# starkware-libs/stark-perpetual

Measured on AMD Instinct MI355X. Metric: pedersen_hashes_per_sec, higher is better.
Workload: dtype u32x9; 1 GPU; 2^16-leaf Pedersen Merkle rebuild per GPU (BASELINE.json configs[1]), 63 rebuilds in lockstep; tree_height=16, leaves_per_gpu=65536, calls_per_region=28, streams=2, window_bits=26, combine=none

## Files before the change

### stark-perpetual_amd/csrc/pedersen.hip

```cpp
#include <cstdlib>
#include <cstring>
#include <map>
#include <vector>

#include "context.hpp"
#include "quad.hpp"

#ifndef SP_ACC_WAVES
#define SP_ACC_WAVES 1
#endif

namespace sp {

struct raw_aff {
  u256 x, y;
};
__device__ __forceinline__ raw_aff ld_raw(const aff_packed* e) {
  const uint4* q = reinterpret_cast<const uint4*>(e);
  const uint4 a = q[0], b = q[1], c = q[2], d = q[3];
  raw_aff r;
  r.x.w[0] = a.x; r.x.w[1] = a.y; r.x.w[2] = a.z; r.x.w[3] = a.w;
  r.x.w[4] = b.x; r.x.w[5] = b.y; r.x.w[6] = b.z; r.x.w[7] = b.w;
  r.y.w[0] = c.x; r.y.w[1] = c.y; r.y.w[2] = c.z; r.y.w[3] = c.w;
  r.y.w[4] = d.x; r.y.w[5] = d.y; r.y.w[6] = d.z; r.y.w[7] = d.w;
  return r;
}
__device__ __forceinline__ aff unpack_raw(const raw_aff& t) {
  aff r;
  r.x = fe_unpack(t.x);
  r.y = fe_unpack(t.y);
  return r;
}

struct bits512 {
  uint32_t w[16];
};
__device__ __forceinline__ bits512 concat_xy(const u256& x, const u256& y) {
  bits512 s;
// ... 35 lines not shown
__device__ __forceinline__ int window_width(int g, int w0, int log2e) { return g == 0 ? w0 : log2e + 1; }
__device__ __forceinline__ int window_start(int g, int w0, int log2e) {
  return g == 0 ? 0 : w0 + (g - 1) * (log2e + 1);
}
__device__ __forceinline__ aff signed_aff(const raw_aff& t, bool negative) {
  aff q = unpack_raw(t);
  if (negative) q.y = fe_neg(q.y);
  return q;
}

__device__ __forceinline__ void store_limbs(int32_t* base, size_t n, size_t e, const fe& v) {
#pragma unroll
  for (int k = 0; k < NL; ++k) base[(size_t)k * n + e] = v.l[k];
}
__device__ __forceinline__ fe load_limbs(const int32_t* base, size_t n, size_t e) {
  fe v;
#pragma unroll
  for (int k = 0; k < NL; ++k) v.l[k] = base[(size_t)k * n + e];
  return v;
}

__device__ __forceinline__ void operand_pointers(const uint64_t* x, const uint64_t* y, size_t xstride,
                                                 size_t ystride, const int2* __restrict__ src, size_t e,
                                                 const uint64_t*& fx, const uint64_t*& fy) {
  if (src == nullptr) {
    fx = x + 4 * e * xstride;
    fy = y + 4 * e * ystride;
  } else {
    const int2 s = src[e];
    fx = s.x >= 0 ? x + 4 * (size_t)s.x : y;
    fy = s.y >= 0 ? x + 4 * (size_t)s.y : y;
  }
}

__device__ __forceinline__ void
bulk_accumulate(const uint64_t* __restrict__ x, const uint64_t* __restrict__ y, size_t xstride,
                size_t ystride, size_t n, const aff_packed* __restrict__ ped, int w0, int log2e,
                int nwin, int32_t* __restrict__ sX, int32_t* __restrict__ sZZ,
                uint8_t* __restrict__ status, unsigned* __restrict__ flag,
                const int2* __restrict__ src, size_t plane, size_t e) {
  if (e >= n) return;
  const uint64_t *fx, *fy;
  operand_pointers(x, y, xstride, ystride, src, e, fx, fy);
  u256 sx = ld_u256(fx);
  u256 sy = ld_u256(fy);
  uint8_t st = SP_HASH_OK;
  if (!u256_lt(sx, U256_P) || !u256_lt(sy, U256_P)) {
    st = SP_HASH_OUT_OF_RANGE;
#pragma unroll
    for (int i = 0; i < 8; ++i) { sx.w[i] = 0; sy.w[i] = 0; }
  }
  bits512 str = concat_xy(sx, sy);
  auto next_window = [&](int g) {
    return window_entry(ped, g, pop_bits(str, window_width(g, w0, log2e)), w0, log2e);
  };
  const raw_aff e0 = ld_raw(next_window(0).entry);
  window_ref r1 = next_window(1 < nwin ? 1 : 0);
  raw_aff n1 = ld_raw(r1.entry);
  bool neg1 = r1.negative, neg2 = false;
  raw_aff n2 = n1;
  if (nwin > 2) {
    const window_ref r2 = next_window(2);
    n2 = ld_raw(r2.entry);
    neg2 = r2.negative;
  }
  xyzz acc;
  int first = 1;
  if (nwin > 2) {
    const aff q1 = signed_aff(n1, neg1);
    n1 = n2;
    neg1 = neg2;
    if (3 < nwin) {
      const window_ref r = next_window(3);
      n2 = ld_raw(r.entry);
      neg2 = r.negative;
    }
    acc = xyzz_mmadd(unpack_raw(e0), q1);
    first = 2;
  } else {
    acc = xyzz_from_aff(unpack_raw(e0));
  }
  for (int i = first; i + 1 < nwin; ++i) {
    const aff q = signed_aff(n1, neg1);
    n1 = n2;
    neg1 = neg2;
    if (i + 2 < nwin) {
      const window_ref r = next_window(i + 2);
      n2 = ld_raw(r.entry);
      neg2 = r.negative;
    }
    acc = xyzz_madd(acc, q);
  }
  if (nwin > 1) {
    fe X3, ZZ3;
    xyzz_madd_x_only(acc, signed_aff(n1, neg1), X3, ZZ3);
    store_limbs(sX, plane, e, X3);
    store_limbs(sZZ, plane, e, ZZ3);
  } else {
    store_limbs(sX, plane, e, acc.X);
    store_limbs(sZZ, plane, e, acc.ZZ);
  }
  if (st != SP_HASH_OK) {
    if (status) status[e] = st;
    if (flag) atomicOr(flag, (unsigned)st);
  } else if (status) {
    status[e] = SP_HASH_OK;
  }
}

__global__ void __launch_bounds__(256, SP_ACC_WAVES)
ped_accumulate_kernel(const uint64_t* __restrict__ x, const uint64_t* __restrict__ y, size_t xstride,
                      size_t ystride, size_t n, const aff_packed* __restrict__ ped, int w0, int log2e,
                      int nwin, int32_t* __restrict__ sX, int32_t* __restrict__ sZZ,
                      uint8_t* __restrict__ status, unsigned* __restrict__ flag,
                      const int2* __restrict__ src, size_t plane) {
  bulk_accumulate(x, y, xstride, ystride, n, ped, w0, log2e, nwin, sX, sZZ, status, flag, src, plane,
                  (size_t)blockIdx.x * blockDim.x + threadIdx.x);
}

__device__ __forceinline__ fe shfl_xor_fe(const fe& v, int mask) {
  fe r;
#pragma unroll
  for (int i = 0; i < NL; ++i) r.l[i] = __shfl_xor(v.l[i], mask, 64);
  return r;
}
__device__ __forceinline__ uint32_t field_from_memory(const uint64_t* felt, int bit, int width) {
  const uint32_t* w = reinterpret_cast<const uint32_t*>(felt);
  const int wi = bit >> 5, sh = bit & 31;
// ... 2 lines not shown
  return (uint32_t)(two >> sh) & ((1u << width) - 1u);
}
__device__ __forceinline__ uint32_t window_from_memory(const uint64_t* fx, const uint64_t* fy, int start,
                                                       int width) {
  if (start + width <= 252) return field_from_memory(fx, start, width);
  if (start >= 252) return field_from_memory(fy, start - 252, width);
  const int lo_n = 252 - start;
  return field_from_memory(fx, start, lo_n) | (field_from_memory(fy, 0, width - lo_n) << lo_n);
}

template <int LOG_L>
__device__ __forceinline__ xyzz split_accumulate(const uint64_t* fx, const uint64_t* fy, int sub,
                                                 const aff_packed* __restrict__ ped, int w0, int log2e,
                                                 int nwin) {
  constexpr int L = 1 << LOG_L;
  const int cnt_lo = nwin / L, extra = nwin % L;
  const int cnt = cnt_lo + (sub < extra ? 1 : 0);
  const int g0 = sub * cnt_lo + (sub < extra ? sub : extra);
  auto entry = [&](int g) {
    return window_entry(ped, g, window_from_memory(fx, fy, window_start(g, w0, log2e), window_width(g, w0, log2e)),
                        w0, log2e);
  };
  const window_ref r0 = entry(g0);
  const aff q0 = signed_aff(ld_raw(r0.entry), r0.negative);
  window_ref rn = entry(g0 + 1);
  raw_aff nxt = ld_raw(rn.entry);
  xyzz acc;
  {
    const aff q1 = signed_aff(nxt, rn.negative);
    if (cnt > 2) {
      rn = entry(g0 + 2);
      nxt = ld_raw(rn.entry);
    }
    acc = xyzz_mmadd(q0, q1);
  }
  for (int j = 2; j < cnt; ++j) {
    const aff q = signed_aff(nxt, rn.negative);
    if (j + 1 < cnt) {
      rn = entry(g0 + j + 1);
      nxt = ld_raw(rn.entry);
    }
    acc = xyzz_madd(acc, q);
  }
#pragma unroll 1
  for (int r = 0; r + 1 < LOG_L; ++r) {
    xyzz o;
    o.X = shfl_xor_fe(acc.X, 1 << r);
    o.Y = shfl_xor_fe(acc.Y, 1 << r);
    o.ZZ = shfl_xor_fe(acc.ZZ, 1 << r);
    o.ZZZ = shfl_xor_fe(acc.ZZZ, 1 << r);
    acc = xyzz_add(acc, o);
  }
  if constexpr (LOG_L > 0) {
    constexpr int r = LOG_L - 1;
    xyzz o;
    o.X = shfl_xor_fe(acc.X, 1 << r);
    o.Y = shfl_xor_fe(acc.Y, 1 << r);
    o.ZZ = shfl_xor_fe(acc.ZZ, 1 << r);
    o.ZZZ = shfl_xor_fe(acc.ZZZ, 1 << r);
    fe X3, ZZ3;
    xyzz_add_x_only(acc, o, X3, ZZ3);
    acc.X = X3;
    acc.ZZ = ZZ3;
  }
  return acc;
}

template <int LOG_L, bool FUSED>
__global__ void __launch_bounds__(256)
ped_accumulate_split_kernel(const uint64_t* __restrict__ x, const uint64_t* __restrict__ y, size_t xstride,
                            size_t ystride, size_t n, const aff_packed* __restrict__ ped, int w0, int log2e,
                            int nwin, int32_t* __restrict__ sX, int32_t* __restrict__ sZZ,
                            uint8_t* __restrict__ status, unsigned* __restrict__ flag,
                            const int2* __restrict__ src, uint64_t* __restrict__ out, size_t ostride,
                            size_t plane) {
  constexpr int L = 1 << LOG_L;
  const size_t gt = (size_t)blockIdx.x * blockDim.x + threadIdx.x;
  const size_t e_raw = gt >> LOG_L;
  const int sub = (int)(gt & (L - 1));
  const bool active = e_raw < n;
  const size_t e = active ? e_raw : n - 1;
  const uint64_t *fx, *fy;
  operand_pointers(x, y, xstride, ystride, src, e, fx, fy);
  const xyzz acc = split_accumulate<LOG_L>(fx, fy, sub, ped, w0, log2e, nwin);
  uint8_t st = SP_HASH_OK;
  u256 xa_plain;
  if (FUSED) {
    fe zz = acc.ZZ;
    if constexpr (LOG_L < 2) {
      if (fe_is_zero(zz)) {
        zz = FE_ONE_M;
        st = SP_HASH_UNHASHABLE;
      }
    }
    const fe zinv = fe_inv_shared_quad<(LOG_L >= 2 ? 0 : 2 - LOG_L), true>(zz, (int)(threadIdx.x & 3));
    if constexpr (LOG_L >= 2) {
      if (limbs_is_zero(zinv)) st = SP_HASH_UNHASHABLE;
    }
    xa_plain = fe_pack(fe_canon(fe_mul(acc.X, zinv)));
  }
  if (!active || sub != 0) return;
  if (!u256_lt(ld_u256(fx), U256_P) || !u256_lt(ld_u256(fy), U256_P)) st = SP_HASH_OUT_OF_RANGE;
  if (FUSED) {
    st_u256(out + 4 * e * ostride, xa_plain);
  } else {
    store_limbs(sX, plane, e, acc.X);
    store_limbs(sZZ, plane, e, acc.ZZ);
  }
  if (status) status[e] = st;
  if (st != SP_HASH_OK && flag) atomicOr(flag, (unsigned)st);
}

template <int LOG_L>
__global__ void __launch_bounds__(256, SP_ACC_WAVES)
ped_accumulate_mixed_kernel(const uint64_t* __restrict__ x, const uint64_t* __restrict__ y, size_t xstride,
                            size_t ystride, size_t n_bulk, size_t rem, unsigned bulk_blocks,
                            const aff_packed* __restrict__ ped, int w0, int log2e, int nwin,
                            int32_t* __restrict__ sX, int32_t* __restrict__ sZZ, uint8_t* __restrict__ status,
                            unsigned* __restrict__ flag, const int2* __restrict__ src, size_t plane) {
  if (blockIdx.x < bulk_blocks) {
    bulk_accumulate(x, y, xstride, ystride, n_bulk, ped, w0, log2e, nwin, sX, sZZ, status, flag, src, plane,
                    (size_t)blockIdx.x * blockDim.x + threadIdx.x);
    return;
  }
  constexpr int L = 1 << LOG_L;
  const size_t gt = (size_t)(blockIdx.x - bulk_blocks) * blockDim.x + threadIdx.x;
  const size_t e_raw = gt >> LOG_L;
  const int sub = (int)(gt & (L - 1));
  const bool active = e_raw < rem;
  const size_t e = n_bulk + (active ? e_raw : rem - 1);
  const uint64_t *fx, *fy;
  operand_pointers(x, y, xstride, ystride, src, e, fx, fy);
  const xyzz acc = split_accumulate<LOG_L>(fx, fy, sub, ped, w0, log2e, nwin);
  if (!active || sub != 0) return;
  uint8_t st = SP_HASH_OK;
  if (!u256_lt(ld_u256(fx), U256_P) || !u256_lt(ld_u256(fy), U256_P)) st = SP_HASH_OUT_OF_RANGE;
  store_limbs(sX, plane, e, acc.X);
  store_limbs(sZZ, plane, e, acc.ZZ);
  if (status) status[e] = st;
  if (st != SP_HASH_OK && flag) atomicOr(flag, (unsigned)st);
}

// ... 393 lines not shown
  };
  aff_packed res;
  if (g1 - g0 == 1) {
    const aff a = entry(g0);
    res.x = fe_pack(fe_canon(a.x));
    res.y = fe_pack(fe_canon(a.y));
  } else {
    xyzz acc = xyzz_mmadd(entry(g0), entry(g0 + 1));
    for (int g = g0 + 2; g < g1; ++g) acc = xyzz_madd(acc, entry(g));
    const fe izzz = fe_inv(acc.ZZZ);
    const fe izz = fe_sqr(fe_mul(acc.ZZ, izzz));
    res.x = fe_pack(fe_canon(fe_mul(acc.X, izz)));
    res.y = fe_pack(fe_canon(fe_mul(acc.Y, izzz)));
  }
  uint4* q = reinterpret_cast<uint4*>(out + t);
  q[0] = make_uint4(res.x.w[0], res.x.w[1], res.x.w[2], res.x.w[3]);
  q[1] = make_uint4(res.x.w[4], res.x.w[5], res.x.w[6], res.x.w[7]);
  q[2] = make_uint4(res.y.w[0], res.y.w[1], res.y.w[2], res.y.w[3]);
  q[3] = make_uint4(res.y.w[4], res.y.w[5], res.y.w[6], res.y.w[7]);
}

struct KernelProfile {
  bool enabled = false;
  std::vector<hipEvent_t> ev;
  std::vector<size_t> units;
  size_t used = 0;
};
static KernelProfile g_prof;
static bool g_split_enabled = getenv("STARKPERP_NO_SPLIT") == nullptr;
static bool g_fuse_enabled = getenv("STARKPERP_NO_FUSE") == nullptr;
static bool g_quad_enabled = getenv("STARKPERP_NO_QUAD") == nullptr;
static bool g_quad2_enabled = getenv("STARKPERP_NO_QUAD2") == nullptr;
static bool g_level_split = getenv("STARKPERP_NO_LEVEL_SPLIT") == nullptr;
static bool g_quad_no_dup = getenv("STARKPERP_QUAD_NO_DUP") != nullptr;
static bool g_sparse_enabled = getenv("STARKPERP_NO_SPARSE_LEVELS") == nullptr;
static size_t g_quad_max = getenv("STARKPERP_QUAD_MAX") ? (size_t)atoll(getenv("STARKPERP_QUAD_MAX")) : 2048;
struct Scratch {
  int32_t *X, *ZZ, *Pre;
  unsigned* flag;
};
static std::map<StreamKey, DeviceBuffer> g_stream_scratch;
int get_scratch_public(size_t n, Scratch& s, hipStream_t st);
static int get_scratch(size_t n, Scratch& s, hipStream_t st) { return get_scratch_public(n, s, st); }
int get_scratch_public(size_t n, Scratch& s, hipStream_t st) {
  DeviceBuffer& buf = g_stream_scratch[stream_key(st)];
  const size_t plane = ((9 * n * sizeof(int32_t)) + 255) & ~(size_t)255;
  SP_HIP(buf.reserve(3 * plane + 256));
  char* b = (char*)buf.ptr;
  s.X = (int32_t*)b;
  s.ZZ = (int32_t*)(b + plane);
  s.Pre = (int32_t*)(b + 2 * plane);
  s.flag = (unsigned*)(b + 3 * plane);
  return SP_OK;
}

static size_t g_finish_lanes = getenv("STARKPERP_FINISH_LANES") ? (size_t)atoll(getenv("STARKPERP_FINISH_LANES")) : 65536;
static size_t parse_split_lanes() {
  const char* e = getenv("STARKPERP_SPLIT_LANES");
  long long v = e ? atoll(e) : 65536;
  if (v < 256) v = 256;
  if (v > (1ll << 24)) v = 1ll << 24;
  return ((size_t)v + 255) & ~(size_t)255;
}
static size_t g_split_lanes = parse_split_lanes();
static bool g_finish_lds = getenv("STARKPERP_NO_FINISH_LDS") == nullptr;
static int finish_lds_ready() {
  static std::map<int, int> done;
  int dev = -1;
  if (hipGetDevice(&dev) != hipSuccess) return SP_ERR_HIP;
  auto it = done.find(dev);
  if (it != done.end()) return it->second;
  const int want = 16 * NL * 256 * (int)sizeof(int32_t);
  hipError_t e = hipFuncSetAttribute(reinterpret_cast<const void*>(ped_finish_lds_kernel<true>),
                                     hipFuncAttributeMaxDynamicSharedMemorySize, want);
  if (e == hipSuccess)
    e = hipFuncSetAttribute(reinterpret_cast<const void*>(ped_finish_lds_kernel<false>),
                            hipFuncAttributeMaxDynamicSharedMemorySize, want);
  if (e != hipSuccess) (void)hipGetLastError();
  return done[dev] = (e == hipSuccess ? SP_OK : SP_ERR_HIP);
}
static size_t finish_threads(size_t n) {
  size_t K = (n + g_finish_lanes - 1) / g_finish_lanes;
  if (K < 1) K = 1;
  if (K > 32) K = 32;
  return ((n + K - 1) / K + 3) & ~(size_t)3;
}

void release_pedersen_state() {
  for (auto& kv : g_stream_scratch) kv.second.release();
  g_stream_scratch.clear();
  for (hipEvent_t e : g_prof.ev) (void)hipEventDestroy(e);
  g_prof.ev.clear();
  g_prof.units.clear();
  g_prof.used = 0;
  g_prof.enabled = false;
}

void constant_window_counts(const PedPlan& p, int& cx, int& cy) {
  cx = cy = 0;
  for (int g = 0; g < p.nwin; ++g) {
    if (p.start[g] + p.bits[g] <= 252) ++cx;
    if (p.start[g] >= 252) ++cy;
  }
}
int enqueue_partial_points(const uint64_t* felts, int count, aff_packed* out, hipStream_t st, bool* usable) {
  Context& c = ctx();
  int cx, cy;
  constant_window_counts(c.plan, cx, cy);
  *usable = cx >= 1 && cy >= 1 && count > 0;
  if (!*usable) return SP_OK;
  hipLaunchKernelGGL(ped_partial_kernel, dim3((unsigned)((2 * count + 63) / 64)), dim3(64), 0, st, felts, count, c.ped,
                     (int)c.plan.bits[0], c.plan.log2e, c.plan.nwin, cx, cy, out);
  SP_HIP(hipGetLastError());
  return SP_OK;
}

static int enqueue_pedersen_impl(const uint64_t* x, size_t xs, const uint64_t* y, size_t ys, uint64_t* out,
                                 size_t os, uint8_t* status, unsigned* flag, size_t n, hipStream_t st,
// ... 132 lines not shown
    fused = true;
  } else if (log_l == 0 && !(g_split_enabled && g_fuse_enabled && n <= 65536)) {
    size_t n_bulk = n, rem = 0;
    int rem_l = 0;
    if (g_level_split && g_split_enabled && n > g_split_lanes && (n % g_split_lanes) != 0 &&
        (n % g_split_lanes) * 2 <= g_split_lanes) {
      rem = n % g_split_lanes;
      rem_l = rem * 8 <= g_split_lanes ? 3 : (rem * 4 <= g_split_lanes ? 2 : 1);
      while (rem_l > 0 && nwin < (2 << rem_l)) --rem_l;
      if (rem_l == 0) rem = 0;
      n_bulk = n - rem;
    }
    if (rem == 0) {
      prof = g_prof.enabled && g_prof.used + 2 <= g_prof.ev.size() && n > 65536;
      if (prof) (void)hipEventRecord(g_prof.ev[g_prof.used], st);
      hipLaunchKernelGGL(ped_accumulate_kernel, dim3((unsigned)((n_bulk + 255) / 256)), dim3(256), 0, st, x, y, xs, ys,
                         n_bulk, c.ped, w0, log2e, nwin, s.X, s.ZZ, status, flag, src, n);
    } else {
      const unsigned bulk_blocks = (unsigned)(n_bulk / 256);
      const unsigned rblocks = (unsigned)(((rem << rem_l) + 255) / 256);
#define SP_LAUNCH_MIXED(LOGL)                                                                                     \
  hipLaunchKernelGGL((ped_accumulate_mixed_kernel<LOGL>), dim3(bulk_blocks + rblocks), dim3(256), 0, st, x, y, xs, \
                     ys, n_bulk, rem, bulk_blocks, c.ped, w0, log2e, nwin, s.X, s.ZZ, status, flag, src, n)
      if (rem_l == 3) SP_LAUNCH_MIXED(3);
      else if (rem_l == 2) SP_LAUNCH_MIXED(2);
      else SP_LAUNCH_MIXED(1);
#undef SP_LAUNCH_MIXED
    }
    if (prof) {
      (void)hipEventRecord(g_prof.ev[g_prof.used + 1], st);
      g_prof.units.push_back(n);
      g_prof.used += 2;
    }
  } else {
    const unsigned blocks = (unsigned)(((n << log_l) + 255) / 256);
    fused = g_fuse_enabled && (n << log_l) <= 65536;
#define SP_LAUNCH_SPLIT(LOGL, FUSEDV)                                                                      \
  hipLaunchKernelGGL((ped_accumulate_split_kernel<LOGL, FUSEDV>), dim3(blocks), dim3(256), 0, st, x, y, xs, \
                     ys, n, c.ped, w0, log2e, nwin, s.X, s.ZZ, status, flag, src, out, os, n)
    if (log_l == 0) SP_LAUNCH_SPLIT(0, true);
    else if (log_l == 3) { if (fused) SP_LAUNCH_SPLIT(3, true); else SP_LAUNCH_SPLIT(3, false); }
    else if (log_l == 2) { if (fused) SP_LAUNCH_SPLIT(2, true); else SP_LAUNCH_SPLIT(2, false); }
    else { if (fused) SP_LAUNCH_SPLIT(1, true); else SP_LAUNCH_SPLIT(1, false); }
#undef SP_LAUNCH_SPLIT
  }
  if (!fused) {
    const size_t T = finish_threads(n);
    const unsigned tpb = T >= 256 ? 256 : 64;
    const unsigned blocksB = (unsigned)((T + tpb - 1) / tpb);
    const size_t kmax = (n + T - 1) / T;
    if (g_finish_lds && tpb == 256 && kmax >= 2 && kmax <= 16 && finish_lds_ready() == SP_OK) {
      const bool z_too = kmax <= 8;
      const size_t lds_bytes = kmax * NL * 256 * sizeof(int32_t) * (z_too ? 2 : 1);
      if (z_too) hipLaunchKernelGGL((ped_finish_lds_kernel<true>), dim3(blocksB), dim3(256), lds_bytes, st, s.X, s.ZZ, n, T,
                                    out, os, status, flag, (int)kmax);
      else hipLaunchKernelGGL((ped_finish_lds_kernel<false>), dim3(blocksB), dim3(256), lds_bytes, st, s.X, s.ZZ, n, T,
                              out, os, status, flag, (int)kmax);
    } else {
      hipLaunchKernelGGL(ped_finish_kernel, dim3(blocksB), dim3(tpb), 0, st, s.X, s.ZZ, s.Pre, n, T, out,
                         os, status, flag);
    }
  }
  SP_HIP(hipGetLastError());
  return SP_OK;
}

}

using namespace sp;

extern "C" {

int sp_pedersen_batch_dev(const uint64_t* x, const uint64_t* y, uint64_t* out, uint8_t* status,
                          size_t n, void* stream) {
  CtxByPointer sp_ctx_sel__(x);
  SP_REQUIRE_READY();
  ctx_lock lk(ctx().mu);
  Scratch s;
  int rc = get_scratch(n, s, (hipStream_t)stream);
  if (rc != SP_OK) return rc;
  return enqueue_pedersen(x, 1, y, 1, out, 1, status, nullptr, n, (hipStream_t)stream, s, nullptr);
}

int sp_pedersen_batch(const uint64_t* x, const uint64_t* y, uint64_t* out, uint8_t* status, size_t n) {
  if (ctx_count() > 1 && shard_context() < 0 && n >= SHARD_MIN_ITEMS) {
    return shard_over_contexts(n, [&](size_t off, size_t cnt) {
// ... 288 lines not shown
```

### stark-perpetual_amd/csrc/curve.hpp

```cpp
#pragma once
#include "fp29.hpp"

namespace sp {

struct aff {
  fe x, y;
};
struct xyzz {
  fe X, Y, ZZ, ZZZ;
};
struct jac {
  fe X, Y, Z;
};

SP_HD xyzz xyzz_from_aff(const aff& p) {
  xyzz r;
  r.X = p.x;
  r.Y = p.y;
  r.ZZ = FE_ONE_M;
  r.ZZZ = FE_ONE_M;
  return r;
}

SP_HD xyzz xyzz_madd(const xyzz& a, const aff& q) {
  const fe U2 = fe_mul(q.x, a.ZZ);
  const fe S2 = fe_mul(q.y, a.ZZZ);
  const fe P = fe_sub(U2, a.X);
  const fe R = fe_sub(S2, a.Y);
  const fe PP = fe_sqr(P);
  const fe PPP = fe_mul(P, PP);
  const fe Q = fe_mul(a.X, PP);
  xyzz r;
  r.X = fe_carry(fe_sub(fe_sub(fe_sqr(R), PPP), fe_dbl(Q)));
  r.Y = fe_mul_sub_mul(R, fe_sub(Q, r.X), a.Y, PPP);
  r.ZZ = fe_mul(a.ZZ, PP);
  r.ZZZ = fe_mul(a.ZZZ, PPP);
  return r;
}

SP_HD void xyzz_madd_x_only(const xyzz& a, const aff& q, fe& X3, fe& ZZ3) {
  const fe U2 = fe_mul(q.x, a.ZZ);
  const fe S2 = fe_mul(q.y, a.ZZZ);
  const fe P = fe_sub(U2, a.X);
  const fe R = fe_sub(S2, a.Y);
  const fe PP = fe_sqr(P);
  const fe PPP = fe_mul(P, PP);
  const fe Q = fe_mul(a.X, PP);
  X3 = fe_carry(fe_sub(fe_sub(fe_sqr(R), PPP), fe_dbl(Q)));
  ZZ3 = fe_mul(a.ZZ, PP);
}

SP_HD xyzz xyzz_mmadd(const aff& a, const aff& b) {
  const fe P = fe_sub(b.x, a.x);
  const fe R = fe_carry(fe_sub(b.y, a.y));
  const fe PP = fe_sqr(P);
  const fe PPP = fe_mul(P, PP);
  const fe Q = fe_mul(a.x, PP);
  xyzz r;
  r.X = fe_carry(fe_sub(fe_sub(fe_sqr(R), PPP), fe_dbl(Q)));
  r.Y = fe_mul_sub_mul(R, fe_sub(Q, r.X), a.y, PPP);
  r.ZZ = PP;
  r.ZZZ = PPP;
  return r;
}

SP_HD xyzz xyzz_add(const xyzz& a, const xyzz& b) {
  const fe U1 = fe_mul(a.X, b.ZZ);
  const fe U2 = fe_mul(b.X, a.ZZ);
  const fe S1 = fe_mul(a.Y, b.ZZZ);
  const fe S2 = fe_mul(b.Y, a.ZZZ);
  const fe P = fe_sub(U2, U1);
  const fe R = fe_sub(S2, S1);
  const fe PP = fe_sqr(P);
  const fe PPP = fe_mul(P, PP);
  const fe Q = fe_mul(U1, PP);
  xyzz r;
  r.X = fe_carry(fe_sub(fe_sub(fe_sqr(R), PPP), fe_dbl(Q)));
  r.Y = fe_mul_sub_mul(R, fe_sub(Q, r.X), S1, PPP);
  r.ZZ = fe_mul(fe_mul(a.ZZ, b.ZZ), PP);
  r.ZZZ = fe_mul(fe_mul(a.ZZZ, b.ZZZ), PPP);
  return r;
}

SP_HD void xyzz_add_x_only(const xyzz& a, const xyzz& b, fe& X3, fe& ZZ3) {
  const fe U1 = fe_mul(a.X, b.ZZ);
  const fe U2 = fe_mul(b.X, a.ZZ);
  const fe S1 = fe_mul(a.Y, b.ZZZ);
  const fe S2 = fe_mul(b.Y, a.ZZZ);
  const fe P = fe_sub(U2, U1);
  const fe R = fe_sub(S2, S1);
  const fe PP = fe_sqr(P);
  const fe PPP = fe_mul(P, PP);
  const fe Q = fe_mul(U1, PP);
  X3 = fe_carry(fe_sub(fe_sub(fe_sqr(R), PPP), fe_dbl(Q)));
  ZZ3 = fe_mul(fe_mul(a.ZZ, b.ZZ), PP);
}

SP_HD jac jac_dbl(const jac& p, const fe& a_coef) {
  const fe XX = fe_sqr(p.X);
  const fe YY = fe_sqr(p.Y);
  const fe YYYY = fe_sqr(YY);
  const fe ZZ = fe_sqr(p.Z);
  const fe t0 = fe_carry(fe_add(p.X, YY));
  const fe halfS = fe_carry(fe_sub(fe_sub(fe_sqr(t0), XX), YYYY));
  const fe S = fe_carry(fe_dbl(halfS));
  const fe XX3 = fe_carry(fe_add(fe_dbl(XX), XX));
  const fe M = fe_carry(fe_add(XX3, fe_mul(a_coef, fe_sqr(ZZ))));
  jac r;
  r.X = fe_carry(fe_sub(fe_sqr(M), fe_dbl(S)));
  const fe y4 = fe_carry(fe_dbl(fe_dbl(YYYY)));
  r.Y = fe_carry(fe_sub(fe_mul(M, fe_sub(S, r.X)), fe_dbl(y4)));
  const fe t1 = fe_carry(fe_add(p.Y, p.Z));
  r.Z = fe_carry(fe_sub(fe_sub(fe_sqr(t1), YY), ZZ));
  return r;
}

struct mjac {
  fe X, Y, Z, W;
};
SP_HD mjac mjac_from(const jac& p, const fe& a_coef) {
  mjac m;
  m.X = p.X; m.Y = p.Y; m.Z = p.Z;
  m.W = fe_mul(a_coef, fe_sqr(fe_sqr(p.Z)));
  return m;
}
SP_HD void mjac_dbl(mjac& p, bool need_w) {
  const fe XX = fe_sqr(p.X);
  const fe YY = fe_sqr(p.Y);
// ... 53 lines not shown
```

### stark-perpetual_amd/csrc/fp29.hpp

```cpp
#pragma once
#include <stdint.h>

#if defined(__HIPCC__)
#include <hip/hip_runtime.h>
#define SP_HD __host__ __device__ __forceinline__
#else
#define SP_HD inline
#endif

#if defined(SP_CHECK_BOUNDS) && !defined(__HIPCC__)
#include <stdio.h>
#include <stdlib.h>
#define SP_CHK32(expr64)                                                        \
  do {                                                                          \
    long long v__ = (long long)(expr64);                                        \
    if (v__ > 2147483647LL || v__ < -2147483648LL) {                            \
      fprintf(stderr, "limb overflow at %s:%d\n", __FILE__, __LINE__);          \
      abort();                                                                  \
    }                                                                           \
  } while (0)
#define SP_CHK64(expr128)                                                       \
  do {                                                                          \
    __int128 v__ = (expr128);                                                   \
    if (v__ > (__int128)9223372036854775807LL || v__ < -(__int128)9223372036854775807LL) { \
      fprintf(stderr, "column overflow at %s:%d\n", __FILE__, __LINE__);        \
      abort();                                                                  \
    }                                                                           \
  } while (0)
#else
#define SP_CHK32(e) ((void)0)
#define SP_CHK64(e) ((void)0)
#endif

namespace sp {
// ... 194 lines not shown
  cols t;
  cols_zero(t);
  cols_mac(t, a, b);
  return fe_reduce(t);
}
SP_HD fe fe_sqr(const fe& a) {
  cols t;
  cols_zero(t);
  cols_sqr(t, a);
  return fe_reduce(t);
}
SP_HD fe fe_mul_sub_mul(const fe& a, const fe& b, const fe& c, const fe& d) {
  cols t;
  cols_zero(t);
  cols_mac(t, a, b);
  cols_msub(t, c, d);
  return fe_reduce(t);
}
SP_HD fe fe_mul_add_mul(const fe& a, const fe& b, const fe& c, const fe& d) {
  cols t;
  cols_zero(t);
  cols_mac(t, a, b);
  cols_mac(t, c, d);
  return fe_reduce(t);
}

SP_HD fe fe_mul3_add(const fe& a, const fe& b, const fe& c, const fe& d, const fe& e, const fe& f) {
  cols t;
  cols_zero(t);
  cols_mac(t, a, b);
  cols_mac(t, c, d);
  cols_mac(t, e, f);
  return fe_reduce(t);
}

SP_HD bool fe_geq_p_canon_limbs(const fe& a) {
  const bool gt8 = a.l[8] > P8, eq8 = a.l[8] == P8;
  const bool gt6 = a.l[6] > P6, eq6 = a.l[6] == P6;
  const bool low = (a.l[5] | a.l[4] | a.l[3] | a.l[2] | a.l[1]) != 0 || a.l[0] >= 1;
  return gt8 | (eq8 & ((a.l[7] != 0) | gt6 | (eq6 & low)));
}
SP_HD fe fe_canon(const fe& a_in) {
  fe a;
  {
    const int32_t q = a_in.l[8] >> 19;
    a = a_in;
    a.l[0] -= q;
    a.l[6] -= q * P6;
    a.l[8] -= q * P8;
    a = fe_carry(a);
  }
  const int32_t neg = a.l[8] >> 31;
  a.l[0] += neg & 1;
  a.l[6] += neg & P6;
  a.l[8] += neg & P8;
  a = fe_carry(a);
  const int32_t ge = fe_geq_p_canon_limbs(a) ? -1 : 0;
  a.l[0] -= ge & 1;
  a.l[6] -= ge & P6;
  a.l[8] -= ge & P8;
  return fe_carry(a);
}

SP_HD fe fe_to_mont(const fe& a) { return fe_mul(a, FE_R2); }
SP_HD fe fe_from_mont(const fe& a) {
  cols t;
// ... 583 lines not shown
```

Measured before the change: 968.8 million hashes/s.

## Add three-lane-per-pair accumulate kernel for mid-sized Merkle levels

Adds a fused accumulate kernel that processes two hashes across three lanes, each covering a contiguous run of the combined windows. Partial XYZZ sums are merged via wave shuffles before a shared quad inversion and direct output store. It is chosen for log_l==0 levels where n falls between half and all of the split-lane budget. The goal is to raise lane utilization and avoid the finish kernel on these levels, at the cost of one idle lane per wave, 64-lane shuffles of full points, and select-based control flow. Finish-plan helpers move into a shared header.

```diff
diff --git a/stark-perpetual_amd/csrc/lane_plan.hpp b/stark-perpetual_amd/csrc/lane_plan.hpp
--- /dev/null
+++ b/stark-perpetual_amd/csrc/lane_plan.hpp
@@ -0,0 +1,56 @@
+#pragma once
+#include <cstddef>
+
+#if defined(__HIPCC__)
+#define SP_LP_HD __host__ __device__ __forceinline__
+#else
+#define SP_LP_HD inline
+#endif
+
+namespace sp {
+
+constexpr int TRI_GROUPS_PER_WAVE = 21;
+
+SP_LP_HD int tri_outer_windows(int nwin) { return (2 * nwin + 1) / 3; }
+SP_LP_HD bool tri_plan_ok(int nwin) {
+  const int a = tri_outer_windows(nwin);
+  return a >= 2 && nwin - a >= 2;
+}
+SP_LP_HD void tri_run(int nwin, int sub, int& lo, int& hi) {
+  const int a = tri_outer_windows(nwin);
+  lo = sub == 0 ? 0 : (sub == 1 ? a : 2 * nwin - a);
+  hi = sub == 0 ? a : (sub == 1 ? 2 * nwin - a : 2 * nwin);
+}
+SP_LP_HD int tri_rounds(int nwin) {
+  const int a = tri_outer_windows(nwin);
+  const int outer = a - 1, middle = 2 * (nwin - a) - 2;
+  return outer > middle ? outer : middle;
+}
+SP_LP_HD int tri_window_of_round(int nwin, int sub, int lo, int r) {
+  int c = lo + 1 + r;
+  if (sub == 1 && c >= nwin) ++c;
+  return c;
+}
+SP_LP_HD size_t tri_waves(size_t n) {
+  const size_t pairs = (n + 1) / 2;
+  return (pairs + TRI_GROUPS_PER_WAVE - 1) / TRI_GROUPS_PER_WAVE;
+}
+SP_LP_HD bool tri_plan_wanted(size_t n, int nwin, size_t lanes) {
+  return n <= lanes && 2 * n > lanes && tri_waves(n) * 64 <= lanes && tri_plan_ok(nwin);
+}
+
+SP_LP_HD size_t finish_plan_threads(size_t n, size_t lanes) {
+  size_t K = (n + lanes - 1) / lanes;
+  if (K < 1) K = 1;
+  if (K > 32) K = 32;
+  return ((n + K - 1) / K + 3) & ~(size_t)3;
+}
+constexpr size_t FINISH_LDS_PER_CU = 160 * 1024;
+constexpr int FINISH_BLOCKS_PER_CU = 1;
+SP_LP_HD bool finish_lds_holds_zz(size_t kmax) { return kmax <= 8; }
+SP_LP_HD size_t finish_lds_bytes(size_t kmax) {
+  if (kmax < 2 || kmax > 16) return 0;
+  return kmax * 9 * 256 * sizeof(int) * (finish_lds_holds_zz(kmax) ? 2 : 1);
+}
+
+}
diff --git a/stark-perpetual_amd/csrc/pedersen.hip b/stark-perpetual_amd/csrc/pedersen.hip
--- a/stark-perpetual_amd/csrc/pedersen.hip
+++ b/stark-perpetual_amd/csrc/pedersen.hip
@@ -4,6 +4,7 @@
 #include <vector>
 
 #include "context.hpp"
+#include "lane_plan.hpp"
 #include "quad.hpp"
 
 #ifndef SP_ACC_WAVES
@@ -311,6 +312,106 @@
     store_limbs(sZZ, plane, e, acc.ZZ);
   }
   if (status) status[e] = st;
+  if (st != SP_HASH_OK && flag) atomicOr(flag, (unsigned)st);
+}
+
+__device__ __forceinline__ fe shfl_fe(const fe& v, int lane) {
+  fe r;
+#pragma unroll
+  for (int i = 0; i < NL; ++i) r.l[i] = __shfl(v.l[i], lane, 64);
+  return r;
+}
+__device__ __forceinline__ xyzz shfl_xyzz(const xyzz& v, int lane) {
+  xyzz r;
+  r.X = shfl_fe(v.X, lane);
+  r.Y = shfl_fe(v.Y, lane);
+  r.ZZ = shfl_fe(v.ZZ, lane);
+  r.ZZZ = shfl_fe(v.ZZZ, lane);
+  return r;
+}
+__device__ __forceinline__ xyzz xyzz_sel(bool c, const xyzz& a, const xyzz& b) {
+  xyzz r;
+  r.X = fe_sel(c, a.X, b.X);
+  r.Y = fe_sel(c, a.Y, b.Y);
+  r.ZZ = fe_sel(c, a.ZZ, b.ZZ);
+  r.ZZZ = fe_sel(c, a.ZZZ, b.ZZZ);
+  return r;
+}
+__global__ void __launch_bounds__(256)
+ped_accumulate_tri_kernel(const uint64_t* __restrict__ x, const uint64_t* __restrict__ y, size_t xstride,
+                          size_t ystride, size_t n, const aff_packed* __restrict__ ped, int w0, int log2e, int nwin,
+                          uint8_t* __restrict__ status, unsigned* __restrict__ flag, const int2* __restrict__ src,
+                          uint64_t* __restrict__ out, size_t ostride) {
+  const size_t gt = (size_t)blockIdx.x * blockDim.x + threadIdx.x;
+  const int lane = (int)(threadIdx.x & 63);
+  const int vl = lane == 63 ? 60 : lane;
+  const int grp = vl / 3, sub = vl - 3 * grp;
+  const size_t pair = (gt >> 6) * TRI_GROUPS_PER_WAVE + (size_t)grp;
+  const size_t e0_raw = 2 * pair, e1_raw = 2 * pair + 1;
+  const size_t e0 = e0_raw < n ? e0_raw : n - 1;
+  const size_t e1 = e1_raw < n ? e1_raw : n - 1;
+  const uint64_t *fx0, *fy0, *fx1, *fy1;
+  operand_pointers(x, y, xstride, ystride, src, e0, fx0, fy0);
+  operand_pointers(x, y, xstride, ystride, src, e1, fx1, fy1);
+  int lo, hi;
+  tri_run(nwin, sub, lo, hi);
+  const int rounds = tri_rounds(nwin);
+  const bool mid = sub == 1;
+  auto entry = [&](int c) {
+    const bool second = c >= nwin;
+    const int g = second ? c - nwin : c;
+    const uint64_t* fx = second ? fx1 : fx0;
+    const uint64_t* fy = second ? fy1 : fy0;
+    return window_entry(ped, g, window_from_memory(fx, fy, window_start(g, w0, log2e), window_width(g, w0, log2e)),
+                        w0, log2e);
+  };
+  auto window_of = [&](int r) {
+    const int c = tri_window_of_round(nwin, sub, lo, r);
+    return c < hi ? c : hi - 1;
+  };
+  const window_ref r0 = entry(lo);
+  const window_ref rs = entry(mid ? nwin : lo);
+  window_ref rn = entry(window_of(0));
+  const raw_aff t0 = ld_raw(r0.entry), ts = ld_raw(rs.entry);
+  raw_aff nxt = ld_raw(rn.entry);
+  xyzz acc = xyzz_from_aff(signed_aff(t0, r0.negative));
+  const xyzz fresh = xyzz_from_aff(signed_aff(ts, rs.negative));
+  xyzz first = acc;
+#pragma unroll 1
+  for (int r = 0; r < rounds; ++r) {
+    const int c = tri_window_of_round(nwin, sub, lo, r);
+    const aff q = signed_aff(nxt, rn.negative);
+    if (r + 1 < rounds) {
+      rn = entry(window_of(r + 1));
+      nxt = ld_raw(rn.entry);
+    }
+    const bool change = mid && c == nwin + 1;
+    first = xyzz_sel(change, acc, first);
+    const xyzz sum = xyzz_madd(xyzz_sel(change, fresh, acc), q);
+    acc = xyzz_sel(c < hi, sum, acc);
+  }
+  const int base = 3 * grp;
+  const xyzz o1 = shfl_xyzz(first, base + 1);
+  const xyzz o2 = shfl_xyzz(acc, mid ? base : base + 1);
+  const xyzz pa = xyzz_sel(mid, o2, acc);
+  const xyzz pb = xyzz_sel(sub == 0, o1, xyzz_sel(mid, first, o2));
+  fe X3, ZZ3;
+  xyzz_add_x_only(pa, pb, X3, ZZ3);
+  uint8_t st = SP_HASH_OK;
+  if (fe_is_zero(ZZ3)) {
+    ZZ3 = FE_ONE_M;
+    st = SP_HASH_UNHASHABLE;
+  }
+  const fe zinv = fe_inv_shared_quad<2, true>(ZZ3, (int)(threadIdx.x & 3));
+  const u256 xa_plain = fe_pack(fe_canon(fe_mul(X3, zinv)));
+  if (lane == 63 || mid) return;
+  const size_t e_raw = sub == 0 ? e0_raw : e1_raw;
+  if (e_raw >= n) return;
+  const uint64_t* fx = sub == 0 ? fx0 : fx1;
+  const uint64_t* fy = sub == 0 ? fy0 : fy1;
+  if (!u256_lt(ld_u256(fx), U256_P) || !u256_lt(ld_u256(fy), U256_P)) st = SP_HASH_OUT_OF_RANGE;
+  st_u256(out + 4 * e_raw * ostride, xa_plain);
+  if (status) status[e_raw] = st;
   if (st != SP_HASH_OK && flag) atomicOr(flag, (unsigned)st);
 }
 
@@ -770,6 +871,7 @@
 static bool g_quad_enabled = getenv("STARKPERP_NO_QUAD") == nullptr;
 static bool g_quad2_enabled = getenv("STARKPERP_NO_QUAD2") == nullptr;
 static bool g_level_split = getenv("STARKPERP_NO_LEVEL_SPLIT") == nullptr;
+static bool g_tri_enabled = getenv("STARKPERP_NO_TRI_LANES") == nullptr;
 static bool g_quad_no_dup = getenv("STARKPERP_QUAD_NO_DUP") != nullptr;
 static bool g_sparse_enabled = getenv("STARKPERP_NO_SPARSE_LEVELS") == nullptr;
 static size_t g_quad_max = getenv("STARKPERP_QUAD_MAX") ? (size_t)atoll(getenv("STARKPERP_QUAD_MAX")) : 2048;
@@ -808,7 +910,7 @@
   if (hipGetDevice(&dev) != hipSuccess) return SP_ERR_HIP;
   auto it = done.find(dev);
   if (it != done.end()) return it->second;
-  const int want = 16 * NL * 256 * (int)sizeof(int32_t);
+  const int want = (int)finish_lds_bytes(16);
   hipError_t e = hipFuncSetAttribute(reinterpret_cast<const void*>(ped_finish_lds_kernel<true>),
                                      hipFuncAttributeMaxDynamicSharedMemorySize, want);
   if (e == hipSuccess)
@@ -818,10 +920,7 @@
   return done[dev] = (e == hipSuccess ? SP_OK : SP_ERR_HIP);
 }
 static size_t finish_threads(size_t n) {
-  size_t K = (n + g_finish_lanes - 1) / g_finish_lanes;
-  if (K < 1) K = 1;
-  if (K > 32) K = 32;
-  return ((n + K - 1) / K + 3) & ~(size_t)3;
+  return finish_plan_threads(n, g_finish_lanes);
 }
 
 void release_pedersen_state() {
@@ -1020,6 +1119,11 @@
       g_prof.units.push_back(n);
       g_prof.used += 2;
     }
+  } else if (log_l == 0 && g_tri_enabled && tri_plan_wanted(n, nwin, g_split_lanes)) {
+    const unsigned blocks = (unsigned)((tri_waves(n) + 3) / 4);
+    hipLaunchKernelGGL(ped_accumulate_tri_kernel, dim3(blocks), dim3(256), 0, st, x, y, xs, ys, n, c.ped, w0, log2e, nwin,
+                       status, flag, src, out, os);
+    fused = true;
   } else {
     const unsigned blocks = (unsigned)(((n << log_l) + 255) / 256);
     fused = g_fuse_enabled && (n << log_l) <= 65536;
@@ -1037,9 +1141,9 @@
     const unsigned tpb = T >= 256 ? 256 : 64;
     const unsigned blocksB = (unsigned)((T + tpb - 1) / tpb);
     const size_t kmax = (n + T - 1) / T;
-    if (g_finish_lds && tpb == 256 && kmax >= 2 && kmax <= 16 && finish_lds_ready() == SP_OK) {
-      const bool z_too = kmax <= 8;
-      const size_t lds_bytes = kmax * NL * 256 * sizeof(int32_t) * (z_too ? 2 : 1);
+    const size_t lds_bytes = finish_lds_bytes(kmax);
+    if (g_finish_lds && tpb == 256 && lds_bytes != 0 && finish_lds_ready() == SP_OK) {
+      const bool z_too = finish_lds_holds_zz(kmax);
       if (z_too) hipLaunchKernelGGL((ped_finish_lds_kernel<true>), dim3(blocksB), dim3(256), lds_bytes, st, s.X, s.ZZ, n, T,
                                     out, os, status, flag, (int)kmax);
       else hipLaunchKernelGGL((ped_finish_lds_kernel<false>), dim3(blocksB), dim3(256), lds_bytes, st, s.X, s.ZZ, n, T,
```

New measurement: 969.2 million hashes/s, median of 5. No clear change (+0.0%).

## Add interleaved column-scan Montgomery multiplication for bulk XYZZ point additions

Applied to the files above, without the earlier changes.

Adds a column-wise product-scanning field multiply that fuses Montgomery-style reduction into each column (q limbs times the -P6/-P8 constants). It also interleaves several independent multiplications into one scan so their accumulators advance together. The bulk accumulate kernel's madd/mmadd paths use this by default; the split kernel keeps the old path. The aim is more instruction-level parallelism and lower live-register pressure than separate full-column products followed by reduce. The risk is different register allocation and occupancy, and correctness of the bounds depends on the new reduction order.

```diff
diff --git a/stark-perpetual_amd/csrc/curve.hpp b/stark-perpetual_amd/csrc/curve.hpp
--- a/stark-perpetual_amd/csrc/curve.hpp
+++ b/stark-perpetual_amd/csrc/curve.hpp
@@ -22,78 +22,128 @@
   return r;
 }
 
+template <bool SCAN = false>
 SP_HD xyzz xyzz_madd(const xyzz& a, const aff& q) {
-  const fe U2 = fe_mul(q.x, a.ZZ);
-  const fe S2 = fe_mul(q.y, a.ZZZ);
+  if constexpr (SCAN && SP_FE_SCAN) {
+    fe t[3];
+    fe_scan(t, scan_mul{q.x, a.ZZ}, scan_mul{q.y, a.ZZZ});
+    const fe P = fe_sub(t[0], a.X), R = fe_sub(t[1], a.Y);
+    const fe P2 = fe_dbl(P), R2 = fe_dbl(R);
+    fe_scan(t, scan_sqr{P, P2}, scan_sqr{R, R2});
+    const fe PP = t[0], RR = t[1];
+    fe_scan(t, scan_mul{P, PP}, scan_mul{a.X, PP});
+    const fe PPP = t[0], Q = t[1];
+    xyzz r;
+    r.X = fe_carry(fe_sub(fe_sub(RR, PPP), fe_dbl(Q)));
+    const fe D = fe_sub(Q, r.X), nY = fe_neg_pinned(a.Y);
+    fe_scan(t, scan_mul2{R, D, nY, PPP}, scan_mul{a.ZZ, PP}, scan_mul{a.ZZZ, PPP});
+    r.Y = t[0];
+    r.ZZ = t[1];
+    r.ZZZ = t[2];
+    return r;
+  }
+  const fe U2 = fe_mul_t<SCAN>(q.x, a.ZZ);
+  const fe S2 = fe_mul_t<SCAN>(q.y, a.ZZZ);
   const fe P = fe_sub(U2, a.X);
   const fe R = fe_sub(S2, a.Y);
-  const fe PP = fe_sqr(P);
-  const fe PPP = fe_mul(P, PP);
-  const fe Q = fe_mul(a.X, PP);
-  xyzz r;
-  r.X = fe_carry(fe_sub(fe_sub(fe_sqr(R), PPP), fe_dbl(Q)));
-  r.Y = fe_mul_sub_mul(R, fe_sub(Q, r.X), a.Y, PPP);
-  r.ZZ = fe_mul(a.ZZ, PP);
-  r.ZZZ = fe_mul(a.ZZZ, PPP);
-  return r;
-}
-
+  const fe PP = fe_sqr_t<SCAN>(P);
+  const fe PPP = fe_mul_t<SCAN>(P, PP);
+  const fe Q = fe_mul_t<SCAN>(a.X, PP);
+  xyzz r;
+  r.X = fe_carry(fe_sub(fe_sub(fe_sqr_t<SCAN>(R), PPP), fe_dbl(Q)));
+  r.Y = fe_mul_sub_mul_t<SCAN>(R, fe_sub(Q, r.X), a.Y, PPP);
+  r.ZZ = fe_mul_t<SCAN>(a.ZZ, PP);
+  r.ZZZ = fe_mul_t<SCAN>(a.ZZZ, PPP);
+  return r;
+}
+
+template <bool SCAN = false>
 SP_HD void xyzz_madd_x_only(const xyzz& a, const aff& q, fe& X3, fe& ZZ3) {
-  const fe U2 = fe_mul(q.x, a.ZZ);
-  const fe S2 = fe_mul(q.y, a.ZZZ);
+  if constexpr (SCAN && SP_FE_SCAN) {
+    fe t[3];
+    fe_scan(t, scan_mul{q.x, a.ZZ}, scan_mul{q.y, a.ZZZ});
+    const fe P = fe_sub(t[0], a.X), R = fe_sub(t[1], a.Y);
+    const fe P2 = fe_dbl(P), R2 = fe_dbl(R);
+    fe_scan(t, scan_sqr{P, P2}, scan_sqr{R, R2});
+    const fe PP = t[0], RR = t[1];
+    fe_scan(t, scan_mul{P, PP}, scan_mul{a.X, PP}, scan_mul{a.ZZ, PP});
+    X3 = fe_carry(fe_sub(fe_sub(RR, t[0]), fe_dbl(t[1])));
+    ZZ3 = t[2];
+    return;
+  }
+  const fe U2 = fe_mul_t<SCAN>(q.x, a.ZZ);
+  const fe S2 = fe_mul_t<SCAN>(q.y, a.ZZZ);
   const fe P = fe_sub(U2, a.X);
   const fe R = fe_sub(S2, a.Y);
-  const fe PP = fe_sqr(P);
-  const fe PPP = fe_mul(P, PP);
-  const fe Q = fe_mul(a.X, PP);
-  X3 = fe_carry(fe_sub(fe_sub(fe_sqr(R), PPP), fe_dbl(Q)));
-  ZZ3 = fe_mul(a.ZZ, PP);
-}
-
+  const fe PP = fe_sqr_t<SCAN>(P);
+  const fe PPP = fe_mul_t<SCAN>(P, PP);
+  const fe Q = fe_mul_t<SCAN>(a.X, PP);
+  X3 = fe_carry(fe_sub(fe_sub(fe_sqr_t<SCAN>(R), PPP), fe_dbl(Q)));
+  ZZ3 = fe_mul_t<SCAN>(a.ZZ, PP);
+}
+
+template <bool SCAN = false>
 SP_HD xyzz xyzz_mmadd(const aff& a, const aff& b) {
+  if constexpr (SCAN && SP_FE_SCAN) {
+    const fe P = fe_sub(b.x, a.x), R = fe_carry(fe_sub(b.y, a.y));
+    const fe P2 = fe_dbl(P), R2 = fe_dbl(R);
+    fe t[2];
+    fe_scan(t, scan_sqr{P, P2}, scan_sqr{R, R2});
+    const fe PP = t[0], RR = t[1];
+    fe_scan(t, scan_mul{P, PP}, scan_mul{a.x, PP});
+    const fe PPP = t[0], Q = t[1];
+    xyzz r;
+    r.X = fe_carry(fe_sub(fe_sub(RR, PPP), fe_dbl(Q)));
+    r.Y = fe_mul_sub_mul_scan(R, fe_sub(Q, r.X), a.y, PPP);
+    r.ZZ = PP;
+    r.ZZZ = PPP;
+    return r;
+  }
   const fe P = fe_sub(b.x, a.x);
   const fe R = fe_carry(fe_sub(b.y, a.y));
-  const fe PP = fe_sqr(P);
-  const fe PPP = fe_mul(P, PP);
-  const fe Q = fe_mul(a.x, PP);
-  xyzz r;
-  r.X = fe_carry(fe_sub(fe_sub(fe_sqr(R), PPP), fe_dbl(Q)));
-  r.Y = fe_mul_sub_mul(R, fe_sub(Q, r.X), a.y, PPP);
+  const fe PP = fe_sqr_t<SCAN>(P);
+  const fe PPP = fe_mul_t<SCAN>(P, PP);
+  const fe Q = fe_mul_t<SCAN>(a.x, PP);
+  xyzz r;
+  r.X = fe_carry(fe_sub(fe_sub(fe_sqr_t<SCAN>(R), PPP), fe_dbl(Q)));
+  r.Y = fe_mul_sub_mul_t<SCAN>(R, fe_sub(Q, r.X), a.y, PPP);
   r.ZZ = PP;
   r.ZZZ = PPP;
   return r;
 }
 
+template <bool SCAN = false>
 SP_HD xyzz xyzz_add(const xyzz& a, const xyzz& b) {
-  const fe U1 = fe_mul(a.X, b.ZZ);
-  const fe U2 = fe_mul(b.X, a.ZZ);
-  const fe S1 = fe_mul(a.Y, b.ZZZ);
-  const fe S2 = fe_mul(b.Y, a.ZZZ);
+  const fe U1 = fe_mul_t<SCAN>(a.X, b.ZZ);
+  const fe U2 = fe_mul_t<SCAN>(b.X, a.ZZ);
+  const fe S1 = fe_mul_t<SCAN>(a.Y, b.ZZZ);
+  const fe S2 = fe_mul_t<SCAN>(b.Y, a.ZZZ);
   const fe P = fe_sub(U2, U1);
   const fe R = fe_sub(S2, S1);
-  const fe PP = fe_sqr(P);
-  const fe PPP = fe_mul(P, PP);
-  const fe Q = fe_mul(U1, PP);
-  xyzz r;
-  r.X = fe_carry(fe_sub(fe_sub(fe_sqr(R), PPP), fe_dbl(Q)));
-  r.Y = fe_mul_sub_mul(R, fe_sub(Q, r.X), S1, PPP);
-  r.ZZ = fe_mul(fe_mul(a.ZZ, b.ZZ), PP);
-  r.ZZZ = fe_mul(fe_mul(a.ZZZ, b.ZZZ), PPP);
-  return r;
-}
-
+  const fe PP = fe_sqr_t<SCAN>(P);
+  const fe PPP = fe_mul_t<SCAN>(P, PP);
+  const fe Q = fe_mul_t<SCAN>(U1, PP);
+  xyzz r;
+  r.X = fe_carry(fe_sub(fe_sub(fe_sqr_t<SCAN>(R), PPP), fe_dbl(Q)));
+  r.Y = fe_mul_sub_mul_t<SCAN>(R, fe_sub(Q, r.X), S1, PPP);
+  r.ZZ = fe_mul_t<SCAN>(fe_mul_t<SCAN>(a.ZZ, b.ZZ), PP);
+  r.ZZZ = fe_mul_t<SCAN>(fe_mul_t<SCAN>(a.ZZZ, b.ZZZ), PPP);
+  return r;
+}
+
+template <bool SCAN = false>
 SP_HD void xyzz_add_x_only(const xyzz& a, const xyzz& b, fe& X3, fe& ZZ3) {
-  const fe U1 = fe_mul(a.X, b.ZZ);
-  const fe U2 = fe_mul(b.X, a.ZZ);
-  const fe S1 = fe_mul(a.Y, b.ZZZ);
-  const fe S2 = fe_mul(b.Y, a.ZZZ);
+  const fe U1 = fe_mul_t<SCAN>(a.X, b.ZZ);
+  const fe U2 = fe_mul_t<SCAN>(b.X, a.ZZ);
+  const fe S1 = fe_mul_t<SCAN>(a.Y, b.ZZZ);
+  const fe S2 = fe_mul_t<SCAN>(b.Y, a.ZZZ);
   const fe P = fe_sub(U2, U1);
   const fe R = fe_sub(S2, S1);
-  const fe PP = fe_sqr(P);
-  const fe PPP = fe_mul(P, PP);
-  const fe Q = fe_mul(U1, PP);
-  X3 = fe_carry(fe_sub(fe_sub(fe_sqr(R), PPP), fe_dbl(Q)));
-  ZZ3 = fe_mul(fe_mul(a.ZZ, b.ZZ), PP);
+  const fe PP = fe_sqr_t<SCAN>(P);
+  const fe PPP = fe_mul_t<SCAN>(P, PP);
+  const fe Q = fe_mul_t<SCAN>(U1, PP);
+  X3 = fe_carry(fe_sub(fe_sub(fe_sqr_t<SCAN>(R), PPP), fe_dbl(Q)));
+  ZZ3 = fe_mul_t<SCAN>(fe_mul_t<SCAN>(a.ZZ, b.ZZ), PP);
 }
 
 SP_HD jac jac_dbl(const jac& p, const fe& a_coef) {
diff --git a/stark-perpetual_amd/csrc/fp29.hpp b/stark-perpetual_amd/csrc/fp29.hpp
--- a/stark-perpetual_amd/csrc/fp29.hpp
+++ b/stark-perpetual_amd/csrc/fp29.hpp
@@ -1,5 +1,6 @@
 #pragma once
 #include <stdint.h>
+#include <utility>
 
 #if defined(__HIPCC__)
 #include <hip/hip_runtime.h>
@@ -260,6 +261,159 @@
   cols_mac(t, c, d);
   cols_mac(t, e, f);
   return fe_reduce(t);
+}
+
+SP_HD void scan_pin(int64_t& acc) {
+#if defined(__HIP_DEVICE_COMPILE__)
+  asm("" : "+v"(acc));
+#else
+  (void)acc;
+#endif
+}
+SP_HD void scan_mac(int64_t& acc, int32_t a, int32_t b) {
+  SP_CHK64((__int128)acc + (__int128)a * b);
+  acc += (int64_t)a * (int64_t)b;
+  scan_pin(acc);
+}
+SP_HD fe fe_neg_pinned(const fe& a) {
+  fe r = fe_neg(a);
+  fe_pin(r);
+  return r;
+}
+struct scan_mul {
+  static constexpr int STEPS = NL;
+  const fe &a, &b;
+  SP_HD void step(int c, int i, int64_t& acc) const {
+    const int j = c - i;
+    if (j >= 0 && j < NL) scan_mac(acc, a.l[i], b.l[j]);
+  }
+};
+struct scan_sqr {
+  static constexpr int STEPS = NL;
+  const fe &a, &d;
+  SP_HD void step(int c, int i, int64_t& acc) const {
+    const int j = c - i;
+    if (j > i && j < NL) scan_mac(acc, d.l[i], a.l[j]);
+    if (j == i) scan_mac(acc, a.l[i], a.l[i]);
+  }
+};
+struct scan_mul2 {
+  static constexpr int STEPS = 2 * NL;
+  const fe &a, &b, &c, &d;
+  SP_HD void step(int k, int i, int64_t& acc) const {
+    const int j = k - (i % NL);
+    if (j >= 0 && j < NL) scan_mac(acc, i < NL ? a.l[i] : c.l[i - NL], i < NL ? b.l[j] : d.l[j]);
+  }
+};
+struct scan_mul3 {
+  static constexpr int STEPS = 3 * NL;
+  const fe &a, &b, &c, &d, &e, &f;
+  SP_HD void step(int k, int i, int64_t& acc) const {
+    const int j = k - (i % NL);
+    if (j >= 0 && j < NL)
+      scan_mac(acc, i < NL ? a.l[i] : i < 2 * NL ? c.l[i - NL] : e.l[i - 2 * NL], i < NL ? b.l[j] : i < 2 * NL ? d.l[j] : f.l[j]);
+  }
+};
+template <int N>
+struct scan_state {
+  int64_t acc[N];
+  int32_t q[N][NL];
+  int32_t np6, np8;
+};
+constexpr int scan_max(int a) { return a; }
+template <class... T>
+constexpr int scan_max(int a, T... rest) { return a > scan_max(rest...) ? a : scan_max(rest...); }
+template <int COL, int I, int N, class... C>
+SP_HD void scan_round(scan_state<N>& s, const C&... chains) {
+  int k = 0;
+  ((I < C::STEPS ? chains.step(COL, I, s.acc[k]) : (void)0, ++k), ...);
+}
+template <int COL, int N, class... C, int... I>
+SP_HD void scan_column(scan_state<N>& s, fe* r, std::integer_sequence<int, I...>, const C&... chains) {
+  (scan_round<COL, I>(s, chains...), ...);
+  if constexpr (COL >= 6 && COL - 6 < NL) {
+#pragma unroll
+    for (int k = 0; k < N; ++k) scan_mac(s.acc[k], s.q[k][COL - 6], s.np6);
+  }
+  if constexpr (COL >= 8) {
+#pragma unroll
+    for (int k = 0; k < N; ++k) scan_mac(s.acc[k], s.q[k][COL - 8], s.np8);
+  }
+#pragma unroll
+  for (int k = 0; k < N; ++k) {
+    const int32_t lo = (int32_t)((uint32_t)s.acc[k] & LMASK);
+    if constexpr (COL < NL) s.q[k][COL] = lo; else r[k].l[COL - NL] = lo;
+    s.acc[k] >>= LB;
+  }
+}
+template <int N, class... C, int... COL>
+SP_HD void scan_columns(scan_state<N>& s, fe* r, std::integer_sequence<int, COL...>, const C&... chains) {
+  (scan_column<COL>(s, r, std::make_integer_sequence<int, scan_max(C::STEPS...)>(), chains...), ...);
+}
+template <class... C>
+SP_HD void fe_scan(fe* r, const C&... chains) {
+  constexpr int N = sizeof...(C);
+  scan_state<N> s;
+  s.np6 = -P6;
+  s.np8 = -P8;
+#if defined(__HIP_DEVICE_COMPILE__)
+  asm volatile("" : "+s"(s.np6), "+s"(s.np8));
+#endif
+#pragma unroll
+  for (int k = 0; k < N; ++k) s.acc[k] = 0;
+  scan_columns(s, r, std::make_integer_sequence<int, 17>(), chains...);
+#pragma unroll
+  for (int k = 0; k < N; ++k) {
+    SP_CHK32(s.acc[k]);
+    r[k].l[8] = (int32_t)s.acc[k];
+    fe_pin(r[k]);
+  }
+}
+SP_HD fe fe_mul_scan(const fe& a, const fe& b) {
+  fe r;
+  fe_scan(&r, scan_mul{a, b});
+  return r;
+}
+SP_HD fe fe_sqr_scan(const fe& a) {
+  const fe d = fe_dbl(a);
+  fe r;
+  fe_scan(&r, scan_sqr{a, d});
+  return r;
+}
+SP_HD fe fe_mul_sub_mul_scan(const fe& a, const fe& b, const fe& c, const fe& d) {
+  const fe nc = fe_neg_pinned(c);
+  fe r;
+  fe_scan(&r, scan_mul2{a, b, nc, d});
+  return r;
+}
+SP_HD fe fe_mul_add_mul_scan(const fe& a, const fe& b, const fe& c, const fe& d) {
+  fe r;
+  fe_scan(&r, scan_mul2{a, b, c, d});
+  return r;
+}
+SP_HD fe fe_mul3_add_scan(const fe& a, const fe& b, const fe& c, const fe& d, const fe& e, const fe& f) {
+  fe r;
+  fe_scan(&r, scan_mul3{a, b, c, d, e, f});
+  return r;
+}
+
+#ifndef SP_FE_SCAN
+#define SP_FE_SCAN 1
+#endif
+template <bool SCAN>
+SP_HD fe fe_mul_t(const fe& a, const fe& b) {
+  if constexpr (SCAN && SP_FE_SCAN) return fe_mul_scan(a, b);
+  else return fe_mul(a, b);
+}
+template <bool SCAN>
+SP_HD fe fe_sqr_t(const fe& a) {
+  if constexpr (SCAN && SP_FE_SCAN) return fe_sqr_scan(a);
+  else return fe_sqr(a);
+}
+template <bool SCAN>
+SP_HD fe fe_mul_sub_mul_t(const fe& a, const fe& b, const fe& c, const fe& d) {
+  if constexpr (SCAN && SP_FE_SCAN) return fe_mul_sub_mul_scan(a, b, c, d);
+  else return fe_mul_sub_mul(a, b, c, d);
 }
 
 SP_HD bool fe_geq_p_canon_limbs(const fe& a) {
diff --git a/stark-perpetual_amd/csrc/pedersen.hip b/stark-perpetual_amd/csrc/pedersen.hip
--- a/stark-perpetual_amd/csrc/pedersen.hip
+++ b/stark-perpetual_amd/csrc/pedersen.hip
@@ -105,6 +105,13 @@
     fy = s.y >= 0 ? x + 4 * (size_t)s.y : y;
   }
 }
+
+#ifndef SP_SCAN_BULK
+#define SP_SCAN_BULK true
+#endif
+#ifndef SP_SCAN_SPLIT
+#define SP_SCAN_SPLIT false
+#endif
 
 __device__ __forceinline__ void
 bulk_accumulate(const uint64_t* __restrict__ x, const uint64_t* __restrict__ y, size_t xstride,
@@ -148,7 +155,7 @@
       n2 = ld_raw(r.entry);
       neg2 = r.negative;
     }
-    acc = xyzz_mmadd(unpack_raw(e0), q1);
+    acc = xyzz_mmadd<SP_SCAN_BULK>(unpack_raw(e0), q1);
     first = 2;
   } else {
     acc = xyzz_from_aff(unpack_raw(e0));
@@ -162,11 +169,11 @@
       n2 = ld_raw(r.entry);
       neg2 = r.negative;
     }
-    acc = xyzz_madd(acc, q);
+    acc = xyzz_madd<SP_SCAN_BULK>(acc, q);
   }
   if (nwin > 1) {
     fe X3, ZZ3;
-    xyzz_madd_x_only(acc, signed_aff(n1, neg1), X3, ZZ3);
+    xyzz_madd_x_only<SP_SCAN_BULK>(acc, signed_aff(n1, neg1), X3, ZZ3);
     store_limbs(sX, plane, e, X3);
     store_limbs(sZZ, plane, e, ZZ3);
   } else {
@@ -235,7 +242,7 @@
       rn = entry(g0 + 2);
       nxt = ld_raw(rn.entry);
     }
-    acc = xyzz_mmadd(q0, q1);
+    acc = xyzz_mmadd<SP_SCAN_SPLIT>(q0, q1);
   }
   for (int j = 2; j < cnt; ++j) {
     const aff q = signed_aff(nxt, rn.negative);
@@ -243,7 +250,7 @@
       rn = entry(g0 + j + 1);
       nxt = ld_raw(rn.entry);
     }
-    acc = xyzz_madd(acc, q);
+    acc = xyzz_madd<SP_SCAN_SPLIT>(acc, q);
   }
 #pragma unroll 1
   for (int r = 0; r + 1 < LOG_L; ++r) {
@@ -252,7 +259,7 @@
     o.Y = shfl_xor_fe(acc.Y, 1 << r);
     o.ZZ = shfl_xor_fe(acc.ZZ, 1 << r);
     o.ZZZ = shfl_xor_fe(acc.ZZZ, 1 << r);
-    acc = xyzz_add(acc, o);
+    acc = xyzz_add<SP_SCAN_SPLIT>(acc, o);
   }
   if constexpr (LOG_L > 0) {
     constexpr int r = LOG_L - 1;
@@ -262,7 +269,7 @@
     o.ZZ = shfl_xor_fe(acc.ZZ, 1 << r);
     o.ZZZ = shfl_xor_fe(acc.ZZZ, 1 << r);
     fe X3, ZZ3;
-    xyzz_add_x_only(acc, o, X3, ZZ3);
+    xyzz_add_x_only<SP_SCAN_SPLIT>(acc, o, X3, ZZ3);
     acc.X = X3;
     acc.ZZ = ZZ3;
   }
```

New measurement: 955.3 million hashes/s before, 989.8 million hashes/s after (median of 6 runs). +3.6%, better.
